# NVIDIA/nvidia-resiliency-ext

Measured on AMD Instinct MI355X. Metric: generate_report_latency_us, lower is better.
Workload: dtype f32; 1 GPU; 8 ranks x 64 sections x 10000 samples per report, ring capacity 10000, relative+individual scores, gather_on_rank0; logical_ranks_per_gpu=8, rows_per_gpu=512, exchange=none (single process)

## Files before the change

### include/nvrx_straggler.h

```cpp
#ifndef NVRX_STRAGGLER_H
#define NVRX_STRAGGLER_H

#include <stddef.h>
#include <stdint.h>

#ifdef __cplusplus
extern "C" {
#endif

#define NVRX_ABI_VERSION 2

#define NVRX_OK 0
#define NVRX_ERR_INVALID (-22)
#define NVRX_ERR_NOMEM (-12)
#define NVRX_ERR_HIP (-5)
#define NVRX_ERR_STATE (-1)
#define NVRX_ERR_RANGE (-34)
#define NVRX_ERR_TIMEOUT (-62)

#define NVRX_STATS_STRIDE 8
#define NVRX_STAT_MIN 0
#define NVRX_STAT_MAX 1
#define NVRX_STAT_MED 2
#define NVRX_STAT_AVG 3
// ... 20 lines not shown
int nvrx_row_stats(const float *d_samples, const uint32_t *d_counts, const uint8_t *d_kinds, int rows,
                   int row_stride, float *d_stats, void *stream);

int nvrx_score(const float *d_table, int R, int K, int S, int do_indiv, int do_rel,
               const double *thresholds, float *d_scores, uint8_t *d_flags, uint32_t *d_meta,
               uint32_t *d_done_counter, uint32_t seq, const float *d_stats_src, float *d_stats_dst,
               int stats_rows, void *stream);

#define NVRX_ATTR_MAX_TOP 16
#define NVRX_ATTR_SCRATCH_FLOATS(K) (33 * (size_t)(K))
#define NVRX_ATTR_WORDS(n_ranks, top_n) ((size_t)(n_ranks) * 2 * (1 + (size_t)(top_n)) * 4)
int nvrx_attribute(const float *d_table, int R, int K, int S, int first_rank, int n_ranks, int top_n, int do_indiv,
                   int do_rel, float *d_minmed_scratch, void *d_out, void *stream);

int nvrx_row_quantile(const float *d_samples, const uint32_t *d_counts, int rows, int row_stride, uint32_t q_ppm,
                      float *d_out, void *stream);
int nvrx_tail_score(const float *d_tails, const float *d_table, int R, int K, int S, int first_rank, int n_ranks,
                    float *d_colmin_scratch, float *d_out, void *stream);

int nvrx_ctx_create(int device, int local_ranks, int rows_per_rank, int ring_cap, nvrx_ctx **out);
int nvrx_ctx_destroy(nvrx_ctx *ctx);
int nvrx_ctx_set_stream(nvrx_ctx *ctx, void *stream);
int nvrx_ctx_info(const nvrx_ctx *ctx, int what);

int nvrx_row_alloc(nvrx_ctx *ctx, int kind);
int nvrx_row_configure(nvrx_ctx *ctx, int row, int kind, int gid);

int nvrx_ring_push(nvrx_ctx *ctx, int row, float value);
int nvrx_ring_push_many(nvrx_ctx *ctx, int row, const float *values, int n);
int nvrx_ring_push_pairs(nvrx_ctx *ctx, const int32_t *rows, const float *values, int n);
int nvrx_ring_push_staged(nvrx_ctx *ctx, const int32_t *rows, const float *values, int n);
int nvrx_sink_push(void *ctx, const int32_t *rows, const float *values, int n);
int nvrx_sink_row_alloc(void *ctx, int kind);
int nvrx_ring_push_device(nvrx_ctx *ctx, int row, const float *d_values, int n, void *stream);
int nvrx_ring_push_device_rows(nvrx_ctx *ctx, int first_row, int n_rows, const float *d_values, int n, int ld, void *stream);
int nvrx_ring_set_count(nvrx_ctx *ctx, int row, int n);
int nvrx_ring_set_count_all(nvrx_ctx *ctx, int n);
int nvrx_ring_count(const nvrx_ctx *ctx, int row);
int nvrx_ring_counts(const nvrx_ctx *ctx, int32_t *out, int n);
int nvrx_ring_occupancy_changed(nvrx_ctx *ctx, int n);
int nvrx_ring_reset(nvrx_ctx *ctx);
int nvrx_history_reset(nvrx_ctx *ctx, void *stream);
int nvrx_ring_flush(nvrx_ctx *ctx, void *stream);
int nvrx_ring_read(nvrx_ctx *ctx, int row, float *out, int n, void *stream);

int nvrx_event_begin(nvrx_ctx *ctx, int row, void *stream);
// ... 89 lines not shown
```

### nvidia-resiliency-ext_amd/csrc/nvrx_straggler.hip

```cpp
#include <hip/hip_runtime.h>
#include <hip/hip_ext.h>

#include <algorithm>
#include <atomic>
#include <chrono>
#include <thread>
#include <cmath>
#include <cstdarg>
#include <cstdio>
#include <cstdlib>
#include <cstring>
#include <deque>
#include <mutex>
#include <string>
#include <unordered_map>
#include <utility>
#include <vector>

#include "nvrx_straggler.h"

namespace {

thread_local std::string g_err;

// ... 281 lines not shown
    mx = max(mx, dpp0<DPP_QUAD_1032>(mx));
    mn = min(mn, dpp<DPP_QUAD_2301>(0xFFFFFFFFu, mn));
    mx = max(mx, dpp0<DPP_QUAD_2301>(mx));
    mn = min(mn, dpp<DPP_ROW_SHR4>(0xFFFFFFFFu, mn));
    mx = max(mx, dpp0<DPP_ROW_SHR4>(mx));
    mn = min(mn, dpp<DPP_ROW_SHR8>(0xFFFFFFFFu, mn));
    mx = max(mx, dpp0<DPP_ROW_SHR8>(mx));
    mn = min(mn, dpp<DPP_BCAST15>(0xFFFFFFFFu, mn));
    mx = max(mx, dpp0<DPP_BCAST15>(mx));
    mn = min(mn, dpp<DPP_BCAST31>(0xFFFFFFFFu, mn));
    mx = max(mx, dpp0<DPP_BCAST31>(mx));
    mn = (uint32_t)__builtin_amdgcn_readlane((int)mn, 63);
    mx = (uint32_t)__builtin_amdgcn_readlane((int)mx, 63);
}

__device__ __forceinline__ double recip_count(uint32_t c) {
    const double d = (double)c;
    double r = __builtin_amdgcn_rcp(d);
    r = fma(fma(-d, r, 1.0), r, r);
    r = fma(fma(-d, r, 1.0), r, r);
    return c ? r : __builtin_inf();
}

template <int THREADS, int VPT>
__global__ __launch_bounds__(THREADS) void k_row_stats(const float *__restrict__ samples,
                                                       const uint32_t *__restrict__ counts,
                                                       const uint8_t *__restrict__ kinds, int row_stride,
                                                       float *__restrict__ stats, Epilogue ep, int uniform_n) {
    constexpr int WAVES = THREADS / 64;
    constexpr int HIST_BITS = THREADS >= 512 ? NVRX_HIST_BITS_WIDE : 11;
    constexpr int HIST_BINS = 1 << HIST_BITS;
    constexpr int PER = HIST_BINS / THREADS;
    constexpr int G = THREADS / 64;
    constexpr int NKEY = VPT * 4;
    constexpr int CAND_MAX = 256;
    constexpr int CAND_ONE = 64;
    static_assert(HIST_BINS % THREADS == 0, "THREADS must divide the histogram size");
    static_assert(THREADS >= CAND_MAX, "candidate list is initialised one word per thread");

    __shared__ __attribute__((aligned(16))) uint32_t s_hist[HIST_BINS];
    __shared__ __attribute__((aligned(16))) uint32_t s_sum[THREADS];
    __shared__ __attribute__((aligned(16))) uint32_t s_cand[CAND_MAX];
    __shared__ __attribute__((aligned(16))) uint32_t s_lt[CAND_MAX];
    __shared__ __attribute__((aligned(16))) double s_d[2 * WAVES];
    __shared__ __attribute__((aligned(16))) uint32_t s_mm[4];
    __shared__ uint32_t s_cur[1];

    const int row = ep.rows_active ? (int)(blockIdx.x / ep.rows_active) * ep.rows_per_rank + (int)(blockIdx.x % ep.rows_active)
                                   : (int)blockIdx.x;
    const int tid = threadIdx.x;
    const int lane = tid & 63;
    const int wave = tid >> 6;

    NVRX_PHASE(0);
#ifdef NVRX_PHASE_CLOCKS
    if (threadIdx.x == 0 && blockIdx.x < 4096) g_phase[blockIdx.x][10] = wall_clock64();
#endif
    uint32_t n = uniform_n >= 0 ? (uint32_t)uniform_n : counts[row];
    if (n > (uint32_t)row_stride) n = (uint32_t)row_stride;
    const int kind = kinds ? kinds[row] : NVRX_KIND_SECTION;
    const int row_gid = (ep.send && ep.gid) ? ep.gid[row] : -1;
    const float row_hmin = ep.hist_min ? ep.hist_min[row] : __builtin_nanf("");

    float r_min, r_max, r_med, r_avg, r_std;
    int path = 0;

    if (n == 0) {
        r_min = r_max = r_med = r_avg = r_std = __builtin_nanf("");
    } else {
        const float4 *__restrict__ src = reinterpret_cast<const float4 *>(samples + (size_t)row * (size_t)row_stride);
        uint32_t key[NKEY];

        float4 x[VPT];
#pragma unroll
        for (int i = 0; i < VPT; i++) {
            const int v = i * THREADS + tid;
            x[i] = make_float4(0.f, 0.f, 0.f, 0.f);
            if ((uint32_t)(v * 4) < n) x[i] = src[v];
        }
        if constexpr (PER % 4 == 0) {
// ... 433 lines not shown
        NVRX_SUB(9);
    }

    if (tid == 0) {
        float *o = stats + (size_t)row * NVRX_STATS_STRIDE;
        const float weight = n ? (float)n * r_avg : 0.0f;
        o[NVRX_STAT_MIN] = r_min;
        o[NVRX_STAT_MAX] = r_max;
        o[NVRX_STAT_MED] = r_med;
        o[NVRX_STAT_AVG] = r_avg;
        o[NVRX_STAT_STD] = r_std;
        o[NVRX_STAT_NUM] = (float)n;
        o[NVRX_STAT_WEIGHT] = weight;
        o[7] = (float)path;
        float h = row_hmin;
        if (ep.hist_min) {
            if (n && r_med < h) {
                h = r_med;
                ep.hist_min[row] = h;
            }
        }
        if (ep.rowg) {
            unsigned long long *g8 = ep.rowg + (size_t)blockIdx.x * ROW_GRANULES;
            const unsigned long long tag = (unsigned long long)ep.epoch << 32;
            const float vals[ROW_GRANULES] = {n ? r_med : -1.0f, n ? h : __builtin_nanf(""), weight,
                                              r_min, r_max, r_med, r_avg, r_std, (float)n, weight, (float)path};
#pragma unroll
            for (int q = 0; q < ROW_GRANULES; q++)
                __hip_atomic_store(g8 + q, tag | (unsigned long long)__float_as_uint(vals[q]), __ATOMIC_RELAXED,
                                   __HIP_MEMORY_SCOPE_AGENT);
        } else if (ep.send) {
            const int lr = row / ep.rows_per_rank;
            float *s = ep.send + (size_t)lr * ep.L;
            const int g = row_gid;
            if (g >= 0 && g < ep.KS) {
                s[g] = n ? r_med : -1.0f;
                s[ep.KS + g] = n ? h : __builtin_nanf("");
                if (g < ep.K) s[2 * ep.KS + g] = weight;
            }
            if (row - lr * ep.rows_per_rank == 0) s[ep.L - 1] = ep.names_ok;
        }
    }
    NVRX_PHASE(8);
#ifdef NVRX_PHASE_CLOCKS
    if (threadIdx.x == 0 && blockIdx.x < 4096) g_phase[blockIdx.x][9] = wall_clock64();
#endif
}

struct StagedSample {
    uint32_t row_slot;
    float value;
};

__global__ void k_scatter(const uint32_t *__restrict__ h_counts, const StagedSample *__restrict__ h_entries,
                          int n_entries, float *__restrict__ samples, int row_stride,
                          uint32_t *__restrict__ d_counts, int rows, const uint8_t *__restrict__ h_kinds,
                          uint8_t *__restrict__ d_kinds, const int32_t *__restrict__ h_gid,
                          int32_t *__restrict__ d_gid, uint32_t *__restrict__ done_cnt, uint32_t *done_word,
                          uint32_t ticket) {
    const int i = blockIdx.x * blockDim.x + threadIdx.x;
    if (i < n_entries) {
        const StagedSample e = h_entries[i];
        samples[(size_t)(e.row_slot >> 16) * (size_t)row_stride + (e.row_slot & 0xFFFFu)] = e.value;
    }
    if (i < rows) {
        d_counts[i] = h_counts[i];
        if (h_kinds) {
            d_kinds[i] = h_kinds[i];
            d_gid[i] = h_gid[i];
// ... 337 lines not shown
    asm volatile("global_store_dwordx4 %0, %1, off sc0 sc1" : : "v"(dst), "v"(v) : "memory");
}

__host__ __device__ inline size_t score1_lds_bytes(int R, int K, int S) {
    const size_t ks4 = (size_t)((K + S + 3) & ~3);
    const size_t nout = (size_t)R * NVRX_SCORE_LEN(S);
    return ks4 * 4 + ((nout + 3) & ~(size_t)3) * 4 + ((nout + 15) & ~(size_t)15);
}
__host__ __device__ inline size_t score1_table_lds_bytes(int R, int K, int S, int send_floats) {
    return (((size_t)R * NVRX_TABLE_LEN(K, S) + 3) & ~(size_t)3) * 4 + (((size_t)send_floats + 3) & ~(size_t)3) * 4;
}

struct GatherArgs {
    const unsigned long long *g;
    const int32_t *gid;
    float *send;
    nvrx_f4 *stats_out;
    uint32_t *err;
    int n_blocks, rows_active, rows_per_rank, local_ranks;
    float names_ok;
    uint32_t epoch;
    unsigned long long timeout_ticks;
    int poll_naps;
};

__device__ __forceinline__ float wait_granule(const unsigned long long *p, const GatherArgs &g, unsigned long long t0) {
    uint32_t spins = 0;
    for (;;) {
        const unsigned long long x = __hip_atomic_load(p, __ATOMIC_RELAXED, __HIP_MEMORY_SCOPE_AGENT);
        if ((uint32_t)(x >> 32) == g.epoch) return __uint_as_float((uint32_t)x);
        __builtin_amdgcn_s_sleep(2);
        if ((++spins & 0xFFu) == 0u && wall_clock64() - t0 > g.timeout_ticks) {
            __hip_atomic_store(g.err, g.epoch, __ATOMIC_RELAXED, __HIP_MEMORY_SCOPE_SYSTEM);
            return __builtin_nanf("");
        }
    }
}

template <int NTHR>
__global__ __launch_bounds__(NTHR) void k_score1(ScoreArgs a, int fence, PeerArgs pa, GatherArgs ga) {
    extern __shared__ __attribute__((aligned(16))) unsigned char s_raw[];

    const int K = a.K, S = a.S, KS = K + S, R = a.R;
    const int L = NVRX_TABLE_LEN(K, S);
    const int W = NVRX_SCORE_LEN(S);
    const int nout = R * W;
// ... 73 lines not shown
                        got = true;
                    }
                    if (got) {
                        if (slot[c] >= 0) {
                            ga.send[slot[c]] = v;
                            if (s_send) s_send[slot[c]] = v;
                        }
                        pending &= ~(1u << c);
                    }
                }
                if (pending) {
                    for (int nap = 0; nap < ga.poll_naps; nap++) __builtin_amdgcn_s_sleep(1);
                    spins++;
                }
            }
        }
        for (int lr = tid; lr < ga.local_ranks; lr += NTHR) {
            ga.send[(size_t)lr * L + (L - 1)] = ga.names_ok;
            if (s_send) s_send[lr * L + (L - 1)] = ga.names_ok;
        }
        sync();
    }
    const unsigned long long t_rows = wall_clock64();
    if (pa.windows) {
        peer_exchange_block(pa, ga.g ? s_send : nullptr, s_tab);
        __syncthreads();
        if (s_tab) a.table = s_tab;
    } else if (ga.g && s_send) {
        a.table = s_send;
    }
    for (int i = tid; i < a.stats_n4; i += NTHR) {
        const float4 v = a.stats_src[i];
        store16_sys(a.stats_dst + i, nvrx_f4{v.x, v.y, v.z, v.w});
    }
    auto score_all = [&](const float *tab) {
        score_colmin(a, tab, tid, NTHR, s_min);
        if (a.meta && (tid >> 6) == NTHR / 64 - 1) score_meta(a, tab, tid & 63);
        if (tid < nout4 - nout) s_out[nout + tid] = 0.f;
        if (tid < ((nout + 15) & ~15) - nout) s_fl[nout + tid] = 0;
        sync();

        {
            int r = pair_r0, sct = pair_s0;
#pragma unroll 2
            for (int idx = tid; idx < R * S; idx += NTHR) {
                const float *__restrict__ row = tab + (size_t)r * L;
// ... 94 lines not shown
                           __ATOMIC_RELAXED, __HIP_MEMORY_SCOPE_SYSTEM);
        __hip_atomic_store(&a.meta[4], a.seq, __ATOMIC_RELAXED, __HIP_MEMORY_SCOPE_SYSTEM);
    }
    if (ga.g && ga.stats_out) {
        for (int idx = tid; idx < ga.n_blocks * 2; idx += NTHR) {
            const int b = idx >> 1, half = idx & 1;
            const unsigned long long *p = ga.g + (size_t)b * ROW_GRANULES + 3 + 4 * half;
            nvrx_f4 v;
            v.x = wait_granule(p + 0, ga, t_begin);
            v.y = wait_granule(p + 1, ga, t_begin);
            v.z = wait_granule(p + 2, ga, t_begin);
            v.w = wait_granule(p + 3, ga, t_begin);
            const int lr = b / ga.rows_active;
            const int row = lr * ga.rows_per_rank + (b - lr * ga.rows_active);
            store16_sys(ga.stats_out + (size_t)row * 2 + half, v);
        }
        asm volatile("s_waitcnt vmcnt(0)" ::: "memory");
        __syncthreads();
        if (tid == 0 && publish) __hip_atomic_store(&a.meta[5], a.seq, __ATOMIC_RELAXED, __HIP_MEMORY_SCOPE_SYSTEM);
    }
}

using StatsKernel = void (*)(const float *, const uint32_t *, const uint8_t *, int, float *, Epilogue, int);

struct StatsVariant {
    int threads;
    int vpt;
    StatsKernel fn;
};

#define SV(T, V) \
    { T, V, k_row_stats<T, V> }
const StatsVariant kVariants[] = {
    SV(256, 1),  SV(256, 2),  SV(256, 3),  SV(256, 4),  SV(256, 5),   SV(256, 6),  SV(256, 8),  SV(256, 10),
    SV(256, 12), SV(256, 16), SV(512, 1),  SV(512, 2),  SV(512, 3),   SV(512, 4),  SV(512, 5),  SV(512, 6),
    SV(512, 8),  SV(512, 10), SV(512, 12), SV(512, 16), SV(1024, 1),  SV(1024, 2), SV(1024, 3), SV(1024, 4),
    SV(1024, 5), SV(1024, 6), SV(1024, 8), SV(1024, 10), SV(1024, 12), SV(1024, 16),
};
#undef SV

const StatsVariant *pick_variant(int row_stride) {
    int prefs[3] = {512, 1024, 256};
    if (row_stride <= 256 * 4 * 2) {
        prefs[0] = 256;
        prefs[1] = 512;
        prefs[2] = 1024;
    }
    for (int p = 0; p < 3; p++) {
        const StatsVariant *best = nullptr;
        for (const StatsVariant &v : kVariants) {
            if (v.threads != prefs[p]) continue;
            if (v.threads * v.vpt * 4 >= row_stride && (!best || v.vpt < best->vpt)) best = &v;
        }
        if (best) return best;
    }
    return nullptr;
}

int launch_row_stats(const float *d_samples, const uint32_t *d_counts, const uint8_t *d_kinds, int rows,
                     int row_stride, float *d_stats, const Epilogue &ep, hipStream_t stream,
                     hipEvent_t start = nullptr, hipEvent_t stop = nullptr, int uniform_n = -1) {
    if (rows == 0) return NVRX_OK;
    const StatsVariant *v = pick_variant(row_stride);
    if (!v)
        return fail(NVRX_ERR_RANGE, "row_stride %d exceeds the register-resident limit %d", row_stride,
                    NVRX_MAX_RING_CAP);
    if (start || stop) {
        hipExtLaunchKernelGGL(v->fn, dim3(rows), dim3(v->threads), 0, stream, start, stop, 0, d_samples, d_counts,
                              d_kinds, row_stride, d_stats, ep, uniform_n);
    } else {
        hipLaunchKernelGGL(v->fn, dim3(rows), dim3(v->threads), 0, stream, d_samples, d_counts, d_kinds, row_stride,
                           d_stats, ep, uniform_n);
    }
    HIP_TRY(hipGetLastError());
    return NVRX_OK;
}

constexpr int score_single_wg_enabled() { return 1; }
int score_fence_enabled() {
    static int v = -1;
    if (v < 0) {
        const char *e = getenv("NVRX_DEBUG_SCORE_FENCE");
        if (e && *e) {
            v = atoi(e) != 0 ? 1 : 0;
        } else {
            int dev = 0;
            hipDeviceProp_t prop;
            v = 1;
            if (hipGetDevice(&dev) == hipSuccess && hipGetDeviceProperties(&prop, dev) == hipSuccess &&
                (strncmp(prop.gcnArchName, "gfx950", 6) == 0 || strncmp(prop.gcnArchName, "gfx942", 6) == 0))
// ... 134 lines not shown
    bool async_on_ctx = false;
    double last_report_us = 0.0;
    double async_rehome_gap_us = 5000.0;
    hipEvent_t report_ev = nullptr;
    uint64_t report_epoch = 0;
    hipStream_t guard_stream = nullptr;
    bool guard_recorded = true;
    bool stamps_used = false;
    uint64_t guard_done_epoch = 0;
    struct StreamEpoch {
        hipStream_t stream;
        uint64_t epoch;
    };
    std::vector<StreamEpoch> stream_epochs;

    const nvrx_report_desc *attr_desc = nullptr;
    hipStream_t attr_stream = nullptr;
    hipEvent_t attr_ev = nullptr;
    float *attr_scratch = nullptr;
    size_t attr_scratch_elems = 0;

    int tail_uniform_n = -1;

    std::mutex mu;
};

static bool stream_is_capturing(hipStream_t st);
static void stamp_slot_give(int slot);

namespace {

int ctx_set_device(const nvrx_ctx *ctx) {
    HIP_TRY(hipSetDevice(ctx->device));
    return NVRX_OK;
}

inline void mark_side_work(nvrx_ctx *ctx) {
    ctx->side_work = true;
    ctx->side_gen++;
}

int guard_ring_writer(nvrx_ctx *ctx, hipStream_t st) {
    if (!ctx->report_epoch) return NVRX_OK;
    nvrx_ctx::StreamEpoch *se = nullptr;
    for (auto &e : ctx->stream_epochs)
        if (e.stream == st) se = &e;
    if (!se) {
        ctx->stream_epochs.push_back({st, 0});
        se = &ctx->stream_epochs.back();
    }
    if (se->epoch < ctx->report_epoch) {
// ... 302 lines not shown
    HIP_TRY(hipSetDevice(device));

    nvrx_ctx *ctx = new (std::nothrow) nvrx_ctx();
    if (!ctx) return fail(NVRX_ERR_NOMEM, "host allocation failed");
    ctx->device = device;
    ctx->local_ranks = local_ranks;
    ctx->rows_per_rank = rows_per_rank;
    ctx->rows = local_ranks * rows_per_rank;
    ctx->ring_cap = ring_cap;
    ctx->row_stride = (ring_cap + 3) & ~3;
    ctx->stage_cap = 4096;
    ctx->total.assign((size_t)ctx->rows, 0);
    ctx->stage_cnt.assign((size_t)ctx->rows, 0);
    ctx->stage_gen.assign((size_t)ctx->rows, 0);
    ctx->resident_mode = resident_scorer_mode_from_env();
    ctx->poll_naps = poll_naps_from_env();
    {
        const char *e = getenv("NVRX_DEBUG_REPORT_REHOME");
        ctx->rehome_mode = (e && atoi(e) == 0) ? 0 : 1;
        const char *g = getenv("NVRX_DEBUG_ASYNC_REHOME_GAP_US");
        if (g && *g) ctx->async_rehome_gap_us = atof(g);
        const char *eg = getenv("NVRX_DEBUG_EAGER_GUARD");
        ctx->stamps_used = eg && atoi(eg) != 0;
    }

#define CTX_TRY(expr)                                                                         \
    do {                                                                                      \
        hipError_t e_ = (expr);                                                               \
        if (e_ != hipSuccess) {                                                               \
            int rc_ = fail(NVRX_ERR_HIP, "%s failed: %s", #expr, hipGetErrorString(e_));      \
            nvrx_ctx_destroy(ctx);                                                            \
            return rc_;                                                                       \
        }                                                                                     \
    } while (0)

    const size_t nsamp = (size_t)ctx->rows * (size_t)ctx->row_stride;
    CTX_TRY(hipMalloc(reinterpret_cast<void **>(&ctx->d_samples), nsamp * sizeof(float)));
    CTX_TRY(hipMemset(ctx->d_samples, 0, nsamp * sizeof(float)));
    CTX_TRY(hipMalloc(reinterpret_cast<void **>(&ctx->d_counts), (size_t)ctx->rows * sizeof(uint32_t)));
    CTX_TRY(hipMemset(ctx->d_counts, 0, (size_t)ctx->rows * sizeof(uint32_t)));
    CTX_TRY(hipMalloc(reinterpret_cast<void **>(&ctx->d_kinds), (size_t)ctx->rows));
    CTX_TRY(hipMemset(ctx->d_kinds, 0, (size_t)ctx->rows));
    CTX_TRY(hipMalloc(reinterpret_cast<void **>(&ctx->d_gid), (size_t)ctx->rows * sizeof(int32_t)));
    CTX_TRY(hipMemset(ctx->d_gid, 0xFF, (size_t)ctx->rows * sizeof(int32_t)));
    CTX_TRY(hipMalloc(reinterpret_cast<void **>(&ctx->d_hist_min), (size_t)ctx->rows * sizeof(float)));
    hipLaunchKernelGGL(k_fill_f32, dim3((ctx->rows + 255) / 256), dim3(256), 0, nullptr, ctx->d_hist_min, (size_t)ctx->rows, INFINITY);
// ... 27 lines not shown
        const size_t gbytes = 2ull * (size_t)ctx->rows * ROW_GRANULES * sizeof(unsigned long long);
        CTX_TRY(hipMalloc(reinterpret_cast<void **>(&ctx->d_rowg), gbytes));
        CTX_TRY(hipMemset(ctx->d_rowg, 0, gbytes));
        CTX_TRY(hipHostMalloc(reinterpret_cast<void **>(&ctx->h_gather_err), 64, hipHostMallocMapped));
        ctx->h_gather_err[0] = 0;
        CTX_TRY(hipHostGetDevicePointer(reinterpret_cast<void **>(&ctx->d_gather_err), ctx->h_gather_err, 0));
    }
    ctx->stamps_argfree = true;
    if (ctx->stamps_argfree) {
        CTX_TRY(hipGetSymbolAddress(reinterpret_cast<void **>(&ctx->d_stamps), HIP_SYMBOL(g_stamp_slots)));
    } else {
        CTX_TRY(hipMalloc(reinterpret_cast<void **>(&ctx->d_stamps), nvrx_ctx::NSTAMP * sizeof(unsigned long long)));
        CTX_TRY(hipMemset(ctx->d_stamps, 0, nvrx_ctx::NSTAMP * sizeof(unsigned long long)));
    }
    {
        int khz = 0;
        if (hipDeviceGetAttribute(&khz, hipDeviceAttributeWallClockRate, device) == hipSuccess && khz > 0) {
            ctx->us_per_tick = 1000.0f / (float)khz;
            ctx->wall_khz = khz;
        }
    }
    CTX_TRY(hipDeviceSynchronize());
#undef CTX_TRY
    *out = ctx;
    return NVRX_OK;
}

int nvrx_ctx_destroy(nvrx_ctx *ctx) {
    if (!ctx) return NVRX_OK;
    (void)hipSetDevice(ctx->device);
    (void)hipDeviceSynchronize();
    if (ctx->d_samples) (void)hipFree(ctx->d_samples);
    if (ctx->d_counts) (void)hipFree(ctx->d_counts);
    if (ctx->d_kinds) (void)hipFree(ctx->d_kinds);
    if (ctx->d_gid) (void)hipFree(ctx->d_gid);
    if (ctx->d_hist_min) (void)hipFree(ctx->d_hist_min);
    if (ctx->h_bulk) (void)hipHostFree(ctx->h_bulk);
    if (ctx->h_stage_done) (void)hipHostFree(ctx->h_stage_done);
    if (ctx->d_stage_cnt) (void)hipFree(ctx->d_stage_cnt);
    if (ctx->h_kinds) (void)hipHostFree(ctx->h_kinds);
    if (ctx->h_gid) (void)hipHostFree(ctx->h_gid);
    for (StageBuf &b : ctx->buf) {
        if (b.h_counts) (void)hipHostFree(b.h_counts);
        if (b.h_entries) (void)hipHostFree(b.h_entries);
    }
    for (EventPair &p : ctx->pool) {
        (void)hipEventDestroy(p.start);
        (void)hipEventDestroy(p.end);
    }
    for (EventPair &p : ctx->timing_pairs) {
        (void)hipEventDestroy(p.start);
        (void)hipEventDestroy(p.end);
    }
    if (ctx->copy_done) (void)hipEventDestroy(ctx->copy_done);
// ... 25 lines not shown

int nvrx_ctx_set_stream(nvrx_ctx *ctx, void *stream) {
    if (!ctx) return fail(NVRX_ERR_INVALID, "ctx is null");
    std::lock_guard<std::mutex> lk(ctx->mu);
    ctx->default_stream = as_stream(stream);
    return NVRX_OK;
}

int nvrx_ctx_info(const nvrx_ctx *ctx, int what) {
    if (!ctx) return fail(NVRX_ERR_INVALID, "ctx is null");
    switch (what) {
        case 0: return ctx->local_ranks;
        case 1: return ctx->rows_per_rank;
        case 2: return ctx->ring_cap;
        case 3: return ctx->row_stride;
        case 4: return ctx->device;
        case 5: return (int)ctx->reports_rehomed;
        case 6: return ctx->last_rehome_verdict;
        case 7: return (int)ctx->regions_skipped;
        case 8: {
            std::lock_guard<std::mutex> lk(const_cast<nvrx_ctx *>(ctx)->mu);
            return ctx->rows_used;
        }
        default: return fail(NVRX_ERR_INVALID, "unknown info selector %d", what);
    }
}

int nvrx_row_configure(nvrx_ctx *ctx, int row, int kind, int gid) {
    if (!ctx) return fail(NVRX_ERR_INVALID, "ctx is null");
    if (row < 0 || row >= ctx->rows) return fail(NVRX_ERR_INVALID, "row %d out of range [0,%d)", row, ctx->rows);
    if (kind != NVRX_KIND_SECTION && kind != NVRX_KIND_KERNEL) return fail(NVRX_ERR_INVALID, "bad kind %d", kind);
    std::lock_guard<std::mutex> lk(ctx->mu);
    if (ctx->h_kinds[row] != (uint8_t)kind || ctx->h_gid[row] != gid) {
        ctx->h_kinds[row] = (uint8_t)kind;
        ctx->h_gid[row] = gid;
        touch_row(ctx, row);
        ctx->meta_dirty = true;
    }
    return NVRX_OK;
}

int nvrx_row_alloc(nvrx_ctx *ctx, int kind) {
    if (!ctx) return fail(NVRX_ERR_INVALID, "ctx is null");
    if (kind != NVRX_KIND_SECTION && kind != NVRX_KIND_KERNEL) return fail(NVRX_ERR_INVALID, "bad kind %d", kind);
    std::lock_guard<std::mutex> lk(ctx->mu);
    if (ctx->rows_used >= ctx->rows_per_rank)
        return fail(NVRX_ERR_RANGE, "straggler rings are full: %d timing rows per rank", ctx->rows_per_rank);
    const int row = ctx->rows_used++;
// ... 484 lines not shown
        float *dst_cpu = nullptr;
        if (cpu_row >= 0) {
            dst_cpu = ctx->d_samples + (size_t)cpu_row * (size_t)ctx->row_stride + (size_t)(ctx->total[(size_t)cpu_row] % cap);
            ctx->total[(size_t)cpu_row]++;
            touch_row(ctx, cpu_row);
        }
        ctx->counts_dirty = true;
        hipStream_t st = as_stream(stream);
        {
            int grc = guard_ring_writer(ctx, st);
            if (grc) return grc;
        }
        ctx->stamps_used = true;
        hipLaunchKernelGGL(k_stamp_end, dim3(1), dim3(1), 0, st, slot_ptr, ctx->us_per_tick, dst_gpu, dst_cpu, cpu_value);
        HIP_TRY(hipGetLastError());
        if (std::find(ctx->stamp_streams.begin(), ctx->stamp_streams.end(), st) == ctx->stamp_streams.end())
            ctx->stamp_streams.push_back(st);
        return NVRX_OK;
    }
    return fail(NVRX_ERR_STATE, "nvrx_stamp_end(row=%d) without a matching nvrx_stamp_begin", row);
}

static int report_local_impl(nvrx_ctx *ctx, float *d_stats, float *d_send, int K, int S, int names_ok, int rows_active,
                             void *stream, unsigned long long *rowg, uint32_t epoch);

int nvrx_report_local(nvrx_ctx *ctx, float *d_stats, float *d_send, int K, int S, int names_ok, int rows_active,
                      void *stream) {
    if (ctx) {
        std::lock_guard<std::mutex> lk(ctx->mu);
        mark_side_work(ctx);
    }
    return report_local_impl(ctx, d_stats, d_send, K, S, names_ok, rows_active, stream, nullptr, 0);
}

static int report_local_impl(nvrx_ctx *ctx, float *d_stats, float *d_send, int K, int S, int names_ok, int rows_active,
                             void *stream, unsigned long long *rowg, uint32_t epoch) {
    hipStream_t st = as_stream(stream);
    if (!ctx || !d_stats) return fail(NVRX_ERR_INVALID, "null argument");
    if (K < 0 || S < 0) return fail(NVRX_ERR_INVALID, "bad K/S");
    if (rows_active < 0 || rows_active > ctx->rows_per_rank) return fail(NVRX_ERR_INVALID, "rows_active %d outside [0,%d]", rows_active, ctx->rows_per_rank);
    if (rows_active == 0) rows_active = ctx->rows_per_rank;
    std::lock_guard<std::mutex> lk(ctx->mu);
    int rc = ctx_set_device(ctx);
    if (rc) return rc;
    int uniform_n = -1;
    rc = flush_locked(ctx, st, &uniform_n, rows_active);
    if (rc) return rc;
    if (d_send) ctx->tail_uniform_n = uniform_n;
    report_clk(2);
    Epilogue ep{};
    ep.gid = ctx->d_gid;
    ep.hist_min = d_send ? ctx->d_hist_min : nullptr;
    ep.send = d_send;
    ep.rows_per_rank = ctx->rows_per_rank;
    ep.rows_active = rows_active;
    ep.K = K;
    ep.KS = K + S;
    ep.L = NVRX_TABLE_LEN(K, S);
    ep.names_ok = names_ok ? 1.0f : 0.0f;
    ep.rowg = rowg;
    ep.epoch = epoch;
    int pair = -1;
    hipEvent_t ev_start = nullptr, ev_stop = nullptr;
    if (ctx->timing) {
        rc = get_pair(ctx->timing_pairs, ctx->timing_free, &pair);
        if (rc) return rc;
        ev_start = ctx->timing_pairs[(size_t)pair].start;
        ev_stop = ctx->timing_pairs[(size_t)pair].end;
    }
    rc = launch_row_stats(ctx->d_samples, ctx->d_counts, ctx->d_kinds, ctx->local_ranks * rows_active, ctx->row_stride,
                          d_stats, ep, st, ev_start, ev_stop, uniform_n);
    if (rc) return rc;
    if (pair >= 0) ctx->timing_used.push_back(pair);
    report_clk(3);
    return NVRX_OK;
}

struct nvrx_peer {
    int device = 0, world = 0, rank = 0, stride = 0;
    unsigned long long *window = nullptr;
    std::vector<unsigned long long *> mapped;
    std::vector<bool> opened;
    unsigned long long **d_windows = nullptr;
    uint32_t *h_err = nullptr, *d_err = nullptr;
    uint32_t epoch = 0;
    double timeout_s = 1800.0;
    int wall_khz = 100000;
    bool ready = false;
};

static int peer_fill_args(nvrx_peer *p, const void *send, void *recv, size_t count, PeerArgs *a) {
    if (!p || !p->ready || !send || !recv) return fail(NVRX_ERR_INVALID, "peer exchange is not ready");
    if (count == 0 || count > (size_t)p->stride) return fail(NVRX_ERR_RANGE, "%zu floats per rank exceed the window's %d", count, p->stride);
    *a = PeerArgs{};
    a->windows = p->d_windows;
    a->send = static_cast<const float *>(send);
    a->recv = static_cast<float *>(recv);
    a->err = p->d_err;
    a->world = p->world;
    a->rank = p->rank;
    a->count = (int)count;
    a->stride = p->stride;
    p->epoch = (p->epoch % 0x7FFFFFFFu) + 1u;
    a->epoch = p->epoch;
    a->timeout_ticks = (unsigned long long)(p->timeout_s * 1e3 * (double)p->wall_khz);
    return NVRX_OK;
}

int nvrx_report_clocks(double *out8) {
    if (!out8) return fail(NVRX_ERR_INVALID, "null argument");
    memcpy(out8, g_report_clk, sizeof(g_report_clk));
    return NVRX_OK;
}

int nvrx_report(nvrx_ctx *ctx, nvrx_report_desc *d, void *stream) {
    report_clk(0);
    if (!ctx || !d) return fail(NVRX_ERR_INVALID, "null argument");
    if (!d->d_stats || !d->d_send || !d->d_scores || !d->d_meta) return fail(NVRX_ERR_INVALID, "null buffer in the report descriptor");
    const bool exchanging = d->allgather_fn != nullptr;
    if (exchanging && (!d->d_table || d->d_table == d->d_send || d->send_count <= 0))
        return fail(NVRX_ERR_INVALID, "an exchange needs a separate table buffer and a positive send_count");
    const bool is_async = d->h_seq_word == nullptr;
    bool async_gap_ok = false;
    {
        std::lock_guard<std::mutex> lk(ctx->mu);
        const double now_us = g_report_clk[0];
        async_gap_ok = ctx->async_rehome_gap_us > 0.0 && ctx->last_report_us > 0.0 && now_us - ctx->last_report_us >= ctx->async_rehome_gap_us;
        ctx->last_report_us = now_us;
        ctx->last_rehome_verdict = 0;
        if (d->prev_settled) {
            ctx->guard_done_epoch = ctx->report_epoch;
            if (ctx->async_on_ctx && ctx->async_gen == ctx->side_gen) ctx->side_work = false;
            ctx->async_on_ctx = false;
        }
    }
    bool rehomed = false;
    if (ctx->rehome_mode && ((!is_async && !d->guard_rings) || (is_async && d->guard_rings && async_gap_ok))) {
        std::lock_guard<std::mutex> lk(ctx->mu);
// ... 53 lines not shown
                        const long n = strtol(v, nullptr, 10);
                        if (n > 1) high = false;
                        if (n > 1 || strcmp(var, "WORLD_SIZE") == 0) break;
                    }
                }
                if (high) {
                    int least = 0, greatest = 0;
                    HIP_TRY(hipDeviceGetStreamPriorityRange(&least, &greatest));
                    HIP_TRY(hipStreamCreateWithPriority(&ctx->score_stream, hipStreamNonBlocking, greatest));
                } else {
                    HIP_TRY(hipStreamCreateWithFlags(&ctx->score_stream, hipStreamNonBlocking));
                }
            }
            if (d->order_after_enabled && d->order_after_stream != stream)
                HIP_TRY(hipStreamWaitEvent(ctx->score_stream, ctx->order_ev, 0));
            if (!ctx->stamp_streams.empty()) {
                int orc = order_after_stamps(ctx, as_stream(stream), ctx->score_stream);
                if (orc) return orc;
            }
        }
        ctx->gran_epoch = (ctx->gran_epoch % 0x7FFFFFFFu) + 1u;
        unsigned long long *slice = ctx->d_rowg + (size_t)(ctx->gran_epoch & 1u) * (size_t)ctx->rows * ROW_GRANULES;
        int rc2 = report_local_impl(ctx, d->d_stats, d->d_send, d->K, d->S, d->names_ok, d->rows_active, stream, slice,
                                    ctx->gran_epoch);
        if (rc2) return rc2;
        GatherArgs ga{};
        ga.g = slice;
        ga.gid = ctx->d_gid;
        ga.send = d->d_send;
        ga.stats_out = (d->d_stats_dst && d->stats_rows > 0) ? reinterpret_cast<nvrx_f4 *>(d->d_stats_dst) : nullptr;
        ga.err = ctx->d_gather_err;
        ga.n_blocks = rows_launch;
        ga.rows_active = d->rows_active > 0 ? d->rows_active : ctx->rows_per_rank;
        ga.rows_per_rank = ctx->rows_per_rank;
        ga.local_ranks = ctx->local_ranks;
        ga.names_ok = d->names_ok ? 1.0f : 0.0f;
        ga.epoch = ctx->gran_epoch;
        ga.timeout_ticks = (unsigned long long)((d->timeout_s > 0.0 ? d->timeout_s : 1e9) * 1e3 * (double)ctx->wall_khz);
        ga.poll_naps = ctx->poll_naps;
        PeerArgs pa{};
        if (peer_route) {
            rc2 = peer_fill_args(static_cast<nvrx_peer *>(d->comm), d->d_send, d->d_table, (size_t)d->send_count, &pa);
            if (rc2) return rc2;
        }
        d->seq = (d->seq % 0x7FFFFFFFu) + 1u;
        rc2 = score_launch(exchanging ? d->d_table : d->d_send, d->R, d->K, d->S, d->do_indiv, d->do_rel, d->thresholds,
                           d->d_scores, d->d_flags, d->d_meta, d->d_done_counter, d->seq, nullptr, nullptr, 0,
                           ctx->score_stream, peer_route ? &pa : nullptr, &ga);
        if (rc2) return rc2;
        ctx->attr_desc = d, ctx->attr_stream = ctx->score_stream;
        report_clk(4);
        report_clk(5);
        rc2 = nvrx_poll_u32(d->h_seq_word, d->seq, d->timeout_s > 0.0 ? d->timeout_s : 1e30);
        report_clk(6);
        if (rc2) return rc2;
        if (*static_cast<volatile uint32_t *>(ctx->h_gather_err) == ctx->gran_epoch)
            return fail(NVRX_ERR_TIMEOUT, "the score kernel gave up waiting for the statistics kernel's rows (epoch %u)", ctx->gran_epoch);
        if (as_stream(stream) == ctx->default_stream) {
            std::lock_guard<std::mutex> lk(ctx->mu);
            ctx->side_work = false;
            ctx->async_on_ctx = false;
        }
        return NVRX_OK;
    }
    int rc = report_local_impl(ctx, d->d_stats, d->d_send, d->K, d->S, d->names_ok, d->rows_active, stream, nullptr, 0);
    if (rc) return rc;
    if (d->guard_rings) {
        std::lock_guard<std::mutex> lk(ctx->mu);
        ctx->guard_stream = as_stream(stream);
        if (rehomed || !ctx->stamps_used) {
            ctx->guard_recorded = false;
        } else {
            HIP_TRY(hipEventRecord(ctx->report_ev, as_stream(stream)));
            ctx->guard_recorded = true;
        }
        ctx->report_epoch++;
    }
    PeerArgs pa{};
    bool prologue = false;
    if (exchanging && d->allgather_fn == reinterpret_cast<void *>(&nvrx_peer_allgather) &&
        score_fits_single_wg(d->R, d->K, d->S, d->d_scores, d->d_flags) && peer_prologue_enabled()) {
        rc = peer_fill_args(static_cast<nvrx_peer *>(d->comm), d->d_send, d->d_table, (size_t)d->send_count, &pa);
        if (rc) return rc;
        prologue = true;
    } else if (exchanging) {
        using AllGatherFn = int (*)(const void *, void *, size_t, int, void *, void *);
        const int nrc = reinterpret_cast<AllGatherFn>(d->allgather_fn)(d->d_send, d->d_table, (size_t)d->send_count, 7,
                                                                       d->comm, stream);
// ... 353 lines not shown
```

### nvidia-resiliency-ext_amd/nvrx_straggler/_native.py

```python
from __future__ import annotations

import ctypes
import os
import threading
from ctypes import POINTER, c_char_p, c_double, c_float, c_int, c_int32, c_size_t, c_uint32, c_void_p

_LIB_NAME = "libnvrx_straggler_hip.so"
_LIB_PATH = os.path.join(os.environ.get("NVRX_DEBUG_LIB_DIR") or os.path.join(os.path.dirname(os.path.abspath(__file__)), "lib"), _LIB_NAME)

NVRX_ABI_VERSION = 2
STATS_STRIDE = 8
STAT_MIN, STAT_MAX, STAT_MED, STAT_AVG, STAT_STD, STAT_NUM, STAT_WEIGHT = range(7)
KIND_SECTION, KIND_KERNEL = 0, 1
MAX_RING_CAP = 65536
META_WORDS = 8
ERR_TIMEOUT = -62
ERR_RANGE = -34
ERR_INVALID = -22
ATTR_MAX_TOP = 16
TAIL_Q_PPM_MIN, TAIL_Q_PPM_MAX = 500000, 999999



class ReportDesc(ctypes.Structure):
# ... 15 lines not shown

    _fields_ = [
        ("kt_sync", c_void_p), ("kt_hold", c_void_p), ("kt_counter", c_void_p), ("kt_patience_s", c_double),
        ("kt_rows_known", ctypes.c_uint64), ("kt_keys_without_row", ctypes.c_uint64),
        ("rows_used", c_int32), ("asynchronous", c_int32), ("harvest_regions", c_int32), ("out_names_ok", c_int32),
    ]


WINDOW_MISS, WINDOW_NAMES = 1, 2

SYMBOLS = [
    ("nvrx_abi_version", c_int, []),
    ("nvrx_last_error", c_char_p, []),
    ("nvrx_row_stats", c_int, [c_void_p, c_void_p, c_void_p, c_int, c_int, c_void_p, c_void_p]),
    ("nvrx_score", c_int, [c_void_p, c_int, c_int, c_int, c_int, c_int, POINTER(c_double), c_void_p, c_void_p, c_void_p,
                           c_void_p, c_uint32, c_void_p, c_void_p, c_int, c_void_p]),
    ("nvrx_attribute", c_int, [c_void_p, c_int, c_int, c_int, c_int, c_int, c_int, c_int, c_int, c_void_p, c_void_p, c_void_p]),
    ("nvrx_row_quantile", c_int, [c_void_p, c_void_p, c_int, c_int, c_uint32, c_void_p, c_void_p]),
    ("nvrx_tail_score", c_int, [c_void_p, c_void_p, c_int, c_int, c_int, c_int, c_int, c_void_p, c_void_p, c_void_p]),
    ("nvrx_ctx_create", c_int, [c_int, c_int, c_int, c_int, POINTER(c_void_p)]),
    ("nvrx_ctx_destroy", c_int, [c_void_p]),
    ("nvrx_ctx_set_stream", c_int, [c_void_p, c_void_p]),
    ("nvrx_ctx_info", c_int, [c_void_p, c_int]),
    ("nvrx_row_alloc", c_int, [c_void_p, c_int]),
    ("nvrx_row_configure", c_int, [c_void_p, c_int, c_int, c_int]),
    ("nvrx_ring_push", c_int, [c_void_p, c_int, c_float]),
    ("nvrx_ring_push_many", c_int, [c_void_p, c_int, c_void_p, c_int]),
    ("nvrx_ring_push_pairs", c_int, [c_void_p, c_void_p, c_void_p, c_int]),
    ("nvrx_ring_push_staged", c_int, [c_void_p, c_void_p, c_void_p, c_int]),
    ("nvrx_sink_push", c_int, [c_void_p, c_void_p, c_void_p, c_int]),
    ("nvrx_sink_row_alloc", c_int, [c_void_p, c_int]),
    ("nvrx_ring_push_device", c_int, [c_void_p, c_int, c_void_p, c_int, c_void_p]),
    ("nvrx_ring_push_device_rows", c_int, [c_void_p, c_int, c_int, c_void_p, c_int, c_int, c_void_p]),
    ("nvrx_ring_set_count", c_int, [c_void_p, c_int, c_int]),
    ("nvrx_ring_set_count_all", c_int, [c_void_p, c_int]),
    ("nvrx_ring_count", c_int, [c_void_p, c_int]),
    ("nvrx_ring_counts", c_int, [c_void_p, c_void_p, c_int]),
    ("nvrx_ring_occupancy_changed", c_int, [c_void_p, c_int]),
    ("nvrx_window_report", c_int, [c_void_p, c_void_p, c_void_p, c_void_p]),
    ("nvrx_window_clocks", c_int, [POINTER(c_double)]),
    ("nvrx_ring_reset", c_int, [c_void_p]),
    ("nvrx_history_reset", c_int, [c_void_p, c_void_p]),
    ("nvrx_ring_flush", c_int, [c_void_p, c_void_p]),
    ("nvrx_ring_read", c_int, [c_void_p, c_int, c_void_p, c_int, c_void_p]),
    ("nvrx_event_begin", c_int, [c_void_p, c_int, c_void_p]),
    ("nvrx_event_end", c_int, [c_void_p, c_int, c_void_p]),
# ... 110 lines not shown
```

Before: 29.09 us.

## Launch row-stats kernel argument-free from a cached device-resident descriptor

Adds an argument-free variant of the row-stats kernel that reads its pointers and epilogue from a __device__ descriptor. The host uploads the descriptor only when the parameters change, and the gather kernel advances an epoch word that the stats kernel uses to pick the granule slice. The goal is to shrink kernel launch and argument-marshalling cost on the repeated synchronous report path. It adds cross-kernel epoch coupling, a per-device ownership scheme, and a risk of stale descriptors if invalidation is missed.

```diff
diff --git a/include/nvrx_straggler.h b/include/nvrx_straggler.h
--- a/include/nvrx_straggler.h
+++ b/include/nvrx_straggler.h
@@ -66,6 +66,7 @@
 int nvrx_ctx_destroy(nvrx_ctx *ctx);
 int nvrx_ctx_set_stream(nvrx_ctx *ctx, void *stream);
 int nvrx_ctx_info(const nvrx_ctx *ctx, int what);
+int nvrx_debug_stats_desc_invalidate(nvrx_ctx *ctx);
 
 int nvrx_row_alloc(nvrx_ctx *ctx, int kind);
 int nvrx_row_configure(nvrx_ctx *ctx, int row, int kind, int gid);
diff --git a/nvidia-resiliency-ext_amd/csrc/nvrx_straggler.hip b/nvidia-resiliency-ext_amd/csrc/nvrx_straggler.hip
--- a/nvidia-resiliency-ext_amd/csrc/nvrx_straggler.hip
+++ b/nvidia-resiliency-ext_amd/csrc/nvrx_straggler.hip
@@ -327,11 +327,22 @@
     return c ? r : __builtin_inf();
 }
 
-template <int THREADS, int VPT>
-__global__ __launch_bounds__(THREADS) void k_row_stats(const float *__restrict__ samples,
-                                                       const uint32_t *__restrict__ counts,
-                                                       const uint8_t *__restrict__ kinds, int row_stride,
-                                                       float *__restrict__ stats, Epilogue ep, int uniform_n) {
+struct StatsDesc {
+    const float *samples;
+    const uint32_t *counts;
+    const uint8_t *kinds;
+    float *stats;
+    int row_stride;
+    Epilogue ep;
+    int uniform_n;
+    uint32_t epoch;
+};
+__device__ StatsDesc g_stats_desc;
+
+template <int THREADS, int VPT, bool AF = false>
+__device__ __forceinline__ void row_stats_body(const float *__restrict__ samples, const uint32_t *__restrict__ counts,
+                                               const uint8_t *__restrict__ kinds, int row_stride,
+                                               float *__restrict__ stats, Epilogue ep, int uniform_n) {
     constexpr int WAVES = THREADS / 64;
     constexpr int HIST_BITS = THREADS >= 512 ? NVRX_HIST_BITS_WIDE : 11;
     constexpr int HIST_BINS = 1 << HIST_BITS;
@@ -361,6 +372,8 @@
 #ifdef NVRX_PHASE_CLOCKS
     if (threadIdx.x == 0 && blockIdx.x < 4096) g_phase[blockIdx.x][10] = wall_clock64();
 #endif
+    uint32_t af_epoch = 0u;
+    if constexpr (AF) af_epoch = __hip_atomic_load(&g_stats_desc.epoch, __ATOMIC_RELAXED, __HIP_MEMORY_SCOPE_AGENT);
     uint32_t n = uniform_n >= 0 ? (uint32_t)uniform_n : counts[row];
     if (n > (uint32_t)row_stride) n = (uint32_t)row_stride;
     const int kind = kinds ? kinds[row] : NVRX_KIND_SECTION;
@@ -840,7 +853,11 @@
         }
         if (ep.rowg) {
             unsigned long long *g8 = ep.rowg + (size_t)blockIdx.x * ROW_GRANULES;
-            const unsigned long long tag = (unsigned long long)ep.epoch << 32;
+            if constexpr (AF) {
+                const uint32_t rows = (gridDim.x / (uint32_t)ep.rows_active) * (uint32_t)ep.rows_per_rank;
+                g8 += (size_t)(af_epoch & 1u) * (size_t)rows * ROW_GRANULES;
+            }
+            const unsigned long long tag = (unsigned long long)(AF ? af_epoch : ep.epoch) << 32;
             const float vals[ROW_GRANULES] = {n ? r_med : -1.0f, n ? h : __builtin_nanf(""), weight,
                                               r_min, r_max, r_med, r_avg, r_std, (float)n, weight, (float)path};
 #pragma unroll
@@ -863,6 +880,33 @@
 #ifdef NVRX_PHASE_CLOCKS
     if (threadIdx.x == 0 && blockIdx.x < 4096) g_phase[blockIdx.x][9] = wall_clock64();
 #endif
+}
+
+template <int THREADS, int VPT>
+__global__ __launch_bounds__(THREADS) void k_row_stats(const float *__restrict__ samples,
+                                                       const uint32_t *__restrict__ counts,
+                                                       const uint8_t *__restrict__ kinds, int row_stride,
+                                                       float *__restrict__ stats, Epilogue ep, int uniform_n) {
+    row_stats_body<THREADS, VPT>(samples, counts, kinds, row_stride, stats, ep, uniform_n);
+}
+
+template <int THREADS, int VPT>
+__global__ __launch_bounds__(THREADS) void k_row_stats_af() {
+    const StatsDesc __attribute__((address_space(4))) *dp =
+        (const StatsDesc __attribute__((address_space(4))) *)(uintptr_t)&g_stats_desc;
+    Epilogue ep;
+    ep.gid = dp->ep.gid;
+    ep.hist_min = dp->ep.hist_min;
+    ep.send = dp->ep.send;
+    ep.rows_per_rank = dp->ep.rows_per_rank;
+    ep.rows_active = dp->ep.rows_active;
+    ep.K = dp->ep.K;
+    ep.KS = dp->ep.KS;
+    ep.L = dp->ep.L;
+    ep.names_ok = dp->ep.names_ok;
+    ep.rowg = dp->ep.rowg;
+    ep.epoch = 0u;
+    row_stats_body<THREADS, VPT, true>(dp->samples, dp->counts, dp->kinds, dp->row_stride, dp->stats, ep, dp->uniform_n);
 }
 
 struct StagedSample {
@@ -1246,6 +1290,7 @@
     uint32_t epoch;
     unsigned long long timeout_ticks;
     int poll_naps;
+    uint32_t *epoch_word;
 };
 
 __device__ __forceinline__ float wait_granule(const unsigned long long *p, const GatherArgs &g, unsigned long long t0) {
@@ -1365,6 +1410,8 @@
         sync();
     }
     const unsigned long long t_rows = wall_clock64();
+    if (tid == 0 && ga.g && ga.epoch_word)
+        __hip_atomic_store(ga.epoch_word, (ga.epoch % 0x7FFFFFFFu) + 1u, __ATOMIC_RELAXED, __HIP_MEMORY_SCOPE_AGENT);
     if (pa.windows) {
         peer_exchange_block(pa, ga.g ? s_send : nullptr, s_tab);
         __syncthreads();
@@ -1505,15 +1552,17 @@
 }
 
 using StatsKernel = void (*)(const float *, const uint32_t *, const uint8_t *, int, float *, Epilogue, int);
+using StatsKernelAF = void (*)();
 
 struct StatsVariant {
     int threads;
     int vpt;
     StatsKernel fn;
+    StatsKernelAF fn_af;
 };
 
 #define SV(T, V) \
-    { T, V, k_row_stats<T, V> }
+    { T, V, k_row_stats<T, V>, k_row_stats_af<T, V> }
 const StatsVariant kVariants[] = {
     SV(256, 1),  SV(256, 2),  SV(256, 3),  SV(256, 4),  SV(256, 5),   SV(256, 6),  SV(256, 8),  SV(256, 10),
     SV(256, 12), SV(256, 16), SV(512, 1),  SV(512, 2),  SV(512, 3),   SV(512, 4),  SV(512, 5),  SV(512, 6),
@@ -1542,13 +1591,15 @@
 
 int launch_row_stats(const float *d_samples, const uint32_t *d_counts, const uint8_t *d_kinds, int rows,
                      int row_stride, float *d_stats, const Epilogue &ep, hipStream_t stream,
-                     hipEvent_t start = nullptr, hipEvent_t stop = nullptr, int uniform_n = -1) {
+                     hipEvent_t start = nullptr, hipEvent_t stop = nullptr, int uniform_n = -1, bool argfree = false) {
     if (rows == 0) return NVRX_OK;
     const StatsVariant *v = pick_variant(row_stride);
     if (!v)
         return fail(NVRX_ERR_RANGE, "row_stride %d exceeds the register-resident limit %d", row_stride,
                     NVRX_MAX_RING_CAP);
-    if (start || stop) {
+    if (argfree) {
+        hipLaunchKernelGGL(v->fn_af, dim3(rows), dim3(v->threads), 0, stream);
+    } else if (start || stop) {
         hipExtLaunchKernelGGL(v->fn, dim3(rows), dim3(v->threads), 0, stream, start, stop, 0, d_samples, d_counts,
                               d_kinds, row_stride, d_stats, ep, uniform_n);
     } else {
@@ -1729,11 +1780,49 @@
 
     int tail_uniform_n = -1;
 
+    int argfree_mode = 1;
+    bool stats_owner = false;
+    StatsDesc *h_desc = nullptr;
+    StatsDesc *d_desc = nullptr;
+    bool desc_valid = false;
+    uint64_t argfree_launches = 0, desc_uploads = 0;
+
     std::mutex mu;
 };
 
 static bool stream_is_capturing(hipStream_t st);
 static void stamp_slot_give(int slot);
+
+constexpr int STATS_OWNER_DEVICES = 64;
+static std::mutex g_stats_owner_mu;
+static std::atomic<nvrx_ctx *> g_stats_owner[STATS_OWNER_DEVICES];
+
+static void stats_desc_claim(nvrx_ctx *ctx) {
+    if (!ctx->argfree_mode || ctx->stats_owner || ctx->device < 0 || ctx->device >= STATS_OWNER_DEVICES) return;
+    if (g_stats_owner[ctx->device].load(std::memory_order_relaxed)) return;
+    std::lock_guard<std::mutex> lk(g_stats_owner_mu);
+    if (g_stats_owner[ctx->device].load(std::memory_order_relaxed)) return;
+    if (!ctx->h_desc) {
+        if (hipHostMalloc(reinterpret_cast<void **>(&ctx->h_desc), sizeof(StatsDesc), hipHostMallocDefault) != hipSuccess ||
+            hipGetSymbolAddress(reinterpret_cast<void **>(&ctx->d_desc), HIP_SYMBOL(g_stats_desc)) != hipSuccess) {
+            (void)hipGetLastError();
+            ctx->argfree_mode = 0;
+            return;
+        }
+        memset(ctx->h_desc, 0, sizeof(StatsDesc));
+    }
+    ctx->desc_valid = false;
+    ctx->stats_owner = true;
+    g_stats_owner[ctx->device].store(ctx, std::memory_order_relaxed);
+}
+
+static void stats_desc_release(nvrx_ctx *ctx) {
+    if (!ctx->stats_owner) return;
+    std::lock_guard<std::mutex> lk(g_stats_owner_mu);
+    ctx->stats_owner = false;
+    ctx->desc_valid = false;
+    g_stats_owner[ctx->device].store(nullptr, std::memory_order_relaxed);
+}
 
 namespace {
 
@@ -2082,6 +2171,8 @@
         if (g && *g) ctx->async_rehome_gap_us = atof(g);
         const char *eg = getenv("NVRX_DEBUG_EAGER_GUARD");
         ctx->stamps_used = eg && atoi(eg) != 0;
+        const char *af = getenv("NVRX_DEBUG_ARGFREE_STATS");
+        ctx->argfree_mode = (af && *af && atoi(af) == 0) ? 0 : 1;
     }
 
 #define CTX_TRY(expr)                                                                         \
@@ -2155,6 +2246,7 @@
     }
     CTX_TRY(hipDeviceSynchronize());
 #undef CTX_TRY
+    stats_desc_claim(ctx);
     *out = ctx;
     return NVRX_OK;
 }
@@ -2163,6 +2255,8 @@
     if (!ctx) return NVRX_OK;
     (void)hipSetDevice(ctx->device);
     (void)hipDeviceSynchronize();
+    stats_desc_release(ctx);
+    if (ctx->h_desc) (void)hipHostFree(ctx->h_desc);
     if (ctx->d_samples) (void)hipFree(ctx->d_samples);
     if (ctx->d_counts) (void)hipFree(ctx->d_counts);
     if (ctx->d_kinds) (void)hipFree(ctx->d_kinds);
@@ -2234,8 +2328,17 @@
             std::lock_guard<std::mutex> lk(const_cast<nvrx_ctx *>(ctx)->mu);
             return ctx->rows_used;
         }
+        case 9: return (int)ctx->argfree_launches;
+        case 10: return (int)ctx->desc_uploads;
         default: return fail(NVRX_ERR_INVALID, "unknown info selector %d", what);
     }
+}
+
+int nvrx_debug_stats_desc_invalidate(nvrx_ctx *ctx) {
+    if (!ctx) return fail(NVRX_ERR_INVALID, "ctx is null");
+    std::lock_guard<std::mutex> lk(ctx->mu);
+    ctx->desc_valid = false;
+    return NVRX_OK;
 }
 
 int nvrx_row_configure(nvrx_ctx *ctx, int row, int kind, int gid) {
@@ -2766,7 +2869,7 @@
 }
 
 static int report_local_impl(nvrx_ctx *ctx, float *d_stats, float *d_send, int K, int S, int names_ok, int rows_active,
-                             void *stream, unsigned long long *rowg, uint32_t epoch);
+                             void *stream, unsigned long long *rowg, uint32_t epoch, bool sync_report);
 
 int nvrx_report_local(nvrx_ctx *ctx, float *d_stats, float *d_send, int K, int S, int names_ok, int rows_active,
                       void *stream) {
@@ -2774,11 +2877,11 @@
         std::lock_guard<std::mutex> lk(ctx->mu);
         mark_side_work(ctx);
     }
-    return report_local_impl(ctx, d_stats, d_send, K, S, names_ok, rows_active, stream, nullptr, 0);
+    return report_local_impl(ctx, d_stats, d_send, K, S, names_ok, rows_active, stream, nullptr, 0, false);
 }
 
 static int report_local_impl(nvrx_ctx *ctx, float *d_stats, float *d_send, int K, int S, int names_ok, int rows_active,
-                             void *stream, unsigned long long *rowg, uint32_t epoch) {
+                             void *stream, unsigned long long *rowg, uint32_t epoch, bool sync_report) {
     hipStream_t st = as_stream(stream);
     if (!ctx || !d_stats) return fail(NVRX_ERR_INVALID, "null argument");
     if (K < 0 || S < 0) return fail(NVRX_ERR_INVALID, "bad K/S");
@@ -2812,9 +2915,44 @@
         ev_start = ctx->timing_pairs[(size_t)pair].start;
         ev_stop = ctx->timing_pairs[(size_t)pair].end;
     }
+    bool argfree = false;
+    if (sync_report && ctx->argfree_mode && !ctx->timing && !ctx->async_on_ctx) {
+        stats_desc_claim(ctx);
+        if (ctx->stats_owner && !stream_is_capturing(st)) {
+            StatsDesc want;
+            memset(&want, 0, sizeof(want));
+            want.samples = ctx->d_samples;
+            want.counts = ctx->d_counts;
+            want.kinds = ctx->d_kinds;
+            want.stats = d_stats;
+            want.row_stride = ctx->row_stride;
+            want.ep.gid = ep.gid;
+            want.ep.hist_min = ep.hist_min;
+            want.ep.send = ep.send;
+            want.ep.rows_per_rank = ep.rows_per_rank;
+            want.ep.rows_active = ep.rows_active;
+            want.ep.K = ep.K;
+            want.ep.KS = ep.KS;
+            want.ep.L = ep.L;
+            want.ep.names_ok = ep.names_ok;
+            want.ep.rowg = rowg ? ctx->d_rowg : nullptr;
+            want.uniform_n = uniform_n;
+            constexpr size_t taught = offsetof(StatsDesc, epoch);
+            if (ctx->desc_valid && memcmp(ctx->h_desc, &want, taught) == 0) {
+                argfree = true;
+            } else {
+                memcpy(ctx->h_desc, &want, taught);
+                ctx->desc_valid = false;
+                HIP_TRY(hipMemcpyAsync(ctx->d_desc, ctx->h_desc, taught, hipMemcpyHostToDevice, st));
+                ctx->desc_valid = true;
+                ctx->desc_uploads++;
+            }
+        }
+    }
     rc = launch_row_stats(ctx->d_samples, ctx->d_counts, ctx->d_kinds, ctx->local_ranks * rows_active, ctx->row_stride,
-                          d_stats, ep, st, ev_start, ev_stop, uniform_n);
+                          d_stats, ep, st, ev_start, ev_stop, uniform_n, argfree);
     if (rc) return rc;
+    if (argfree) ctx->argfree_launches++;
     if (pair >= 0) ctx->timing_used.push_back(pair);
     report_clk(3);
     return NVRX_OK;
@@ -2857,7 +2995,18 @@
     return NVRX_OK;
 }
 
+static int report_impl(nvrx_ctx *ctx, nvrx_report_desc *d, void *stream);
+
 int nvrx_report(nvrx_ctx *ctx, nvrx_report_desc *d, void *stream) {
+    const int rc = report_impl(ctx, d, stream);
+    if (rc && ctx) {
+        std::lock_guard<std::mutex> lk(ctx->mu);
+        ctx->desc_valid = false;
+    }
+    return rc;
+}
+
+static int report_impl(nvrx_ctx *ctx, nvrx_report_desc *d, void *stream) {
     report_clk(0);
     if (!ctx || !d) return fail(NVRX_ERR_INVALID, "null argument");
     if (!d->d_stats || !d->d_send || !d->d_scores || !d->d_meta) return fail(NVRX_ERR_INVALID, "null buffer in the report descriptor");
@@ -2957,7 +3106,7 @@
         ctx->gran_epoch = (ctx->gran_epoch % 0x7FFFFFFFu) + 1u;
         unsigned long long *slice = ctx->d_rowg + (size_t)(ctx->gran_epoch & 1u) * (size_t)ctx->rows * ROW_GRANULES;
         int rc2 = report_local_impl(ctx, d->d_stats, d->d_send, d->K, d->S, d->names_ok, d->rows_active, stream, slice,
-                                    ctx->gran_epoch);
+                                    ctx->gran_epoch, true);
         if (rc2) return rc2;
         GatherArgs ga{};
         ga.g = slice;
@@ -2973,6 +3122,7 @@
         ga.epoch = ctx->gran_epoch;
         ga.timeout_ticks = (unsigned long long)((d->timeout_s > 0.0 ? d->timeout_s : 1e9) * 1e3 * (double)ctx->wall_khz);
         ga.poll_naps = ctx->poll_naps;
+        ga.epoch_word = ctx->stats_owner ? &ctx->d_desc->epoch : nullptr;
         PeerArgs pa{};
         if (peer_route) {
             rc2 = peer_fill_args(static_cast<nvrx_peer *>(d->comm), d->d_send, d->d_table, (size_t)d->send_count, &pa);
@@ -2998,7 +3148,8 @@
         }
         return NVRX_OK;
     }
-    int rc = report_local_impl(ctx, d->d_stats, d->d_send, d->K, d->S, d->names_ok, d->rows_active, stream, nullptr, 0);
+    int rc = report_local_impl(ctx, d->d_stats, d->d_send, d->K, d->S, d->names_ok, d->rows_active, stream, nullptr, 0,
+                               d->h_seq_word != nullptr);
     if (rc) return rc;
     if (d->guard_rings) {
         std::lock_guard<std::mutex> lk(ctx->mu);
diff --git a/nvidia-resiliency-ext_amd/nvrx_straggler/_native.py b/nvidia-resiliency-ext_amd/nvrx_straggler/_native.py
--- a/nvidia-resiliency-ext_amd/nvrx_straggler/_native.py
+++ b/nvidia-resiliency-ext_amd/nvrx_straggler/_native.py
@@ -61,6 +61,7 @@
     ("nvrx_ctx_destroy", c_int, [c_void_p]),
     ("nvrx_ctx_set_stream", c_int, [c_void_p, c_void_p]),
     ("nvrx_ctx_info", c_int, [c_void_p, c_int]),
+    ("nvrx_debug_stats_desc_invalidate", c_int, [c_void_p]),
     ("nvrx_row_alloc", c_int, [c_void_p, c_int]),
     ("nvrx_row_configure", c_int, [c_void_p, c_int, c_int, c_int]),
     ("nvrx_ring_push", c_int, [c_void_p, c_int, c_float]),
```

Measured after the change: 29.88 us. +2.7%, slower.
